# YHY138/Boosting-Fine-grained-Feature-Fusion-in-3D-Point-Cloud-Registration

Measured on AMD Instinct MI355X. Metric: point-cloud pairs/sec (forward) on ModelNet 2048-pt pairs, higher is better.
Workload: dtype f32 (emulated on the fp16 MFMA pipe: f16x3 split products); 1 GPU; ModelNet40 2048-pt pairs, 8 pairs per GPU (BASELINE configs[1] at N=1, configs[3] at N=8); pairs_per_gpu=8, global_batch=8, points_per_cloud=717, parallelism=pair-sharded dp1, precision=fp32

## Files before the change

### boosting-fine-grained-feature-fusion-in-3d-point-cloud-registration_amd/csrc/res2net.hip

```cpp
#include "mfma.h"

namespace fgr {
namespace {

constexpr int kCpU = 8;
__device__ __forceinline__ void copy_rows(float* __restrict__ dst, int64_t ldd,
                                          const float* __restrict__ src, int64_t lds, int64_t r0,
                                          int rows, int64_t n, int cols, int tid, int nth) {
    const bool v4 = ((cols | (int)(ldd & 3) | (int)(lds & 3)) & 3) == 0 &&
                    ((reinterpret_cast<uintptr_t>(dst) | reinterpret_cast<uintptr_t>(src)) & 15) == 0;
    if (v4) {
        const int c4 = cols / 4;
        const int nr = (int)min<int64_t>(rows, n - r0);
        if (nr <= 0 || c4 == 0) return;
        const int tot = nr * c4;
        for (int e0 = tid; e0 < tot; e0 += kCpU * nth) {
            float4 v[kCpU];
#pragma unroll
            for (int u = 0; u < kCpU; ++u) {
                const int e = min(e0 + u * nth, tot - 1);
                const int row = e / c4, cc = (e - row * c4) * 4;
                v[u] = *reinterpret_cast<const float4*>(src + (r0 + row) * lds + cc);
            }
#pragma unroll
// ... 226 lines not shown
                ah[f] = __builtin_bit_cast(f16x8, img[0 * NU + base + 16 * f + c]);
                am[f] = __builtin_bit_cast(f16x8, img[1 * NU + base + 16 * f + c]);
            }
#pragma unroll
            for (int f = 0; f < RF; ++f) acc[f] = __builtin_amdgcn_mfma_f32_16x16x32_f16(wl, ah[f], acc[f], 0, 0, 0);
#pragma unroll
            for (int f = 0; f < RF; ++f) acc[f] = __builtin_amdgcn_mfma_f32_16x16x32_f16(wh, am[f], acc[f], 0, 0, 0);
#pragma unroll
            for (int f = 0; f < RF; ++f) acc[f] = __builtin_amdgcn_mfma_f32_16x16x32_f16(wh, ah[f], acc[f], 0, 0, 0);
        }
#pragma unroll
        for (int rg = 0; rg < RF; ++rg) {
            const int row = rg * 16 + c;
            const float mx = __int_as_float(rm[row]);
            const float rs = __builtin_ldexpf(1.f, mx > 0.f ? -row_scale_exp(mx) : 0);
            const f32x4 av = acc[rg];
            float4 y;
            y.x = fmaxf(av[0] * rs * wsv.x + bc.x, 0.f);
            y.y = fmaxf(av[1] * rs * wsv.y + bc.y, 0.f);
            y.z = fmaxf(av[2] * rs * wsv.z + bc.z, 0.f);
            y.w = fmaxf(av[3] * rs * wsv.w + bc.w, 0.f);
            if (r0 + row < n && col_ok)
                *reinterpret_cast<float4*>(cat + (r0 + row) * ld + (int64_t)i * w + col0) = y;
            *reinterpret_cast<float4*>(sp + row * SPW + col0) = y;
        }
        if (tid < R) rmax[(i + 1) & 1][tid] = 0;
        __syncthreads();
    }
    copy_rows(cat + (int64_t)nums * w, ld, h + (int64_t)nums * w, hw, r0, R, n,
              (scale - nums) * w, tid, nth);
    if (x) copy_rows(cat + hw, ld, x, cin, r0, R, n, cin, tid, nth);
}

}
}

using namespace fgr;

extern "C" int fgr_res2net_chain_h3(const float* h, int64_t n, int32_t w, int32_t scale,
                                    const void* w_img, const float* w_scale, const float* bias,
                                    const float* x, int32_t cin, float* cat, int64_t ld_cat,
                                    void* stream) {
    FGR_REQUIRE(n >= 0 && scale >= 2 && w > 0 && w <= 224 && w % 4 == 0 && cin >= 0,
                "fgr_res2net_chain_h3: unsupported width %d / scale %d (w %% 4 == 0, <= 224)", w,
                scale);
    FGR_REQUIRE(ld_cat >= (int64_t)scale * w + (x ? cin : 0) && ld_cat % 4 == 0,
                "fgr_res2net_chain_h3: ld_cat too small or not a multiple of 4");
    FGR_REQUIRE(n == 0 || (h && w_img && w_scale && bias && cat), "fgr_res2net_chain_h3: null pointer");
    FGR_REQUIRE(((reinterpret_cast<uintptr_t>(h) | reinterpret_cast<uintptr_t>(cat) |
                  reinterpret_cast<uintptr_t>(w_scale) | reinterpret_cast<uintptr_t>(bias)) & 15) == 0 &&
                    (scale * w) % 4 == 0,
                "fgr_res2net_chain_h3: h / cat / w_scale / bias must be 16-B aligned");
    if (n == 0) return FGR_OK;
    hipStream_t st = as_stream(stream);
    TimedCall timed_(st);
    const int kt = (w + 15) / 16;
    const char* rr = getenv("FGR_R2N_ROWS");
    const bool r48 = kt == 14 && !(rr && rr[0] == '3') &&
                     ceil_div(ceil_div(n, 48), 256) * 48 < ceil_div(ceil_div(n, 32), 256) * 32;
#define FGR_H3_CASE(KT)                                                                         \
    case KT:                                                                                    \
        hipLaunchKernelGGL(res2net_chain_h3_kernel<KT>, dim3((unsigned)ceil_div(n, kRows)),     \
                           dim3(64 * KT), 0, st, h, n, w, scale, scale - 1, (const u32x4*)w_img, \
                           w_scale, bias, x, cin, cat, ld_cat);                                 \
        break;
    if (r48) {
        hipLaunchKernelGGL((res2net_chain_h3_kernel<14, 48>), dim3((unsigned)ceil_div(n, 48)),
                           dim3(64 * 14), 0, st, h, n, w, scale, scale - 1, (const u32x4*)w_img,
                           w_scale, bias, x, cin, cat, ld_cat);
        FGR_CHECK_LAUNCH("res2net_chain_h3_kernel");
// ... 20 lines not shown
                "fgr_res2net_chain6: unsupported width %d / scale %d (needs 112 or 224)", w, scale);
    FGR_REQUIRE(ld_cat >= (int64_t)scale * w + (x ? cin : 0), "fgr_res2net_chain6: ld_cat too small");
    FGR_REQUIRE(n == 0 || (h && w_img && bias && cat), "fgr_res2net_chain6: null pointer");
    FGR_REQUIRE(((reinterpret_cast<uintptr_t>(h) & 15) == 0) && (scale * w) % 4 == 0,
                "fgr_res2net_chain6: h must be 16-B aligned");
    if (n == 0) return FGR_OK;
    hipStream_t st = as_stream(stream);
    TimedCall timed_(st);
    const char* rr = getenv("FGR_R2N_ROWS");
    int rows = 32;
    if (w == 224 && !(rr && rr[0] == '3')) {
        int64_t best = ceil_div(ceil_div(n, 32), 256) * 32;
        for (int r : {48, 16}) {
            const int64_t cost = ceil_div(ceil_div(n, r), 256) * r;
            if (cost < best) { best = cost; rows = r; }
        }
    }
    const int64_t b32 = ceil_div(n, 32);
    if (w == 112)
        hipLaunchKernelGGL(res2net_chain6_kernel<7>, dim3((unsigned)b32), dim3(64 * 7), 0, st, h, n,
                           scale, scale - 1, (const u32x4*)w_img, bias, x, cin, cat, ld_cat);
    else if (rows == 48)
        hipLaunchKernelGGL((res2net_chain6_kernel<14, 48>), dim3((unsigned)ceil_div(n, 48)), dim3(64 * 14),
                           0, st, h, n, scale, scale - 1, (const u32x4*)w_img, bias, x, cin, cat, ld_cat);
    else if (rows == 16)
        hipLaunchKernelGGL((res2net_chain6_kernel<14, 16>), dim3((unsigned)ceil_div(n, 16)), dim3(64 * 14),
                           0, st, h, n, scale, scale - 1, (const u32x4*)w_img, bias, x, cin, cat, ld_cat);
    else
        hipLaunchKernelGGL(res2net_chain6_kernel<14>, dim3((unsigned)b32), dim3(64 * 14), 0, st, h, n,
                           scale, scale - 1, (const u32x4*)w_img, bias, x, cin, cat, ld_cat);
    FGR_CHECK_LAUNCH("res2net_chain6_kernel");
    return FGR_OK;
}
```

### boosting-fine-grained-feature-fusion-in-3d-point-cloud-registration_amd/fgreg/_lib.py

```python
import ctypes
import os
import subprocess

HERE = os.path.dirname(os.path.abspath(__file__))
LIB_PATH = os.environ.get('FGREG_LIB_PATH') or os.path.join(HERE, 'libfgreg.so')
CSRC = os.path.join(os.path.dirname(HERE), 'csrc')

_vp = ctypes.c_void_p
_i32 = ctypes.c_int32
_i64 = ctypes.c_int64
_f32 = ctypes.c_float
_sz = ctypes.c_size_t

ABI_VERSION = 2

SIGNATURES = {
    'fgr_grid_subsample_workspace': [_i64, _i32, _i64, ctypes.POINTER(_sz)],
    'fgr_grid_subsample_count': [_vp, _vp, _i32, _i64, _f32, _i64, _vp, _sz, _vp, _vp],
    'fgr_grid_subsample_fill': [_i64, _i32, _i64, _i64, _vp, _sz, _vp, _vp, _vp, _vp],
    'fgr_radius_grid_workspace': [_i64, _i32, ctypes.POINTER(_sz)],
    'fgr_radius_grid_build': [_vp, _vp, _i32, _i64, _f32, _vp, _sz, _vp],
    'fgr_radius_search_grid': [_vp, _vp, _i32, _i64, _i32, _vp, _vp, _i64, _vp, _sz, _f32, _i32,
                               _i32, _vp, _vp, _vp, _vp],
    'fgr_radius_count': [_vp, _vp, _vp, _vp, _i32, _i64, _i32, _f32, _vp, _vp, _vp],
# ... 6 lines not shown
    'fgr_kpconv_deform_points': [_vp, _vp, _vp, _vp, _i64, _i32, _f32, _vp, _vp, _vp],
    'fgr_kpconv_gather_deform_workspace': [_i64, _i32, ctypes.POINTER(_sz)],
    'fgr_kpconv_gather_deform': [_vp, _vp, _i64, _i64, _vp, _i32, _vp, _i32, _vp, _vp, _i32, _f32,
                                 _i32, _i32, _vp, _vp, _vp, _sz, _vp],
    'fgr_kpconv_scatter_deform_workspace': [_i64, _i32, _i32, ctypes.POINTER(_sz)],
    'fgr_kpconv_scatter_deform': [_vp, _vp, _i64, _i64, _vp, _i32, _vp, _i32, _vp, _vp, _i32, _f32,
                                  _i32, _i32, _vp, _vp, _vp, _vp, _sz, _vp],
    'fgr_kpconv_deform_grad': [_vp, _vp, _i64, _i64, _vp, _i32, _vp, _i32, _vp, _vp, _vp, _i32,
                               _f32, _i32, _i32, _vp, _vp, _vp],
    'fgr_max_pool': [_vp, _i64, _i32, _vp, _i64, _i32, _vp, _vp],
    'fgr_instnorm_workspace': [_i64, _i32, _i32, ctypes.POINTER(_sz)],
    'fgr_instnorm': [_vp, _i64, _i32, _vp, _i32, _i64, _vp, _f32, _i32, _vp, _i32, _vp, _vp, _sz,
                     _vp],
    'fgr_layernorm': [_vp, _i64, _i32, _vp, _vp, _f32, _vp, _vp, _vp, _vp],
    'fgr_sine_pos_embed': [_vp, _i64, _i32, _f32, _f32, _vp, _vp],
    'fgr_add': [_vp, _vp, _i64, _vp, _vp],
    'fgr_layernorm_dual': [_vp, _i64, _i32, _vp, _vp, _vp, _vp, _vp, _vp, _vp, _vp, _f32, _vp],
    'fgr_attention': [_vp, _i64, _vp, _i64, _vp, _i64, _vp, _i64, _vp, _vp, _vp, _i32, _i32, _i32,
                      _i32, _f32, _vp],
    'fgr_attention_f16x3_workspace': [_i64, _i32, _i32, ctypes.POINTER(_sz)],
    'fgr_attention_f16x3': [_vp, _i64, _vp, _i64, _vp, _i64, _vp, _i64, _vp, _vp, _vp, _i32, _i32,
                            _i64, _i32, _i32, _i32, _i32, _f32, _vp, _i64, _vp],
    'fgr_attention_f16x3_drop': [_vp, _i64, _vp, _i64, _vp, _i64, _vp, _i64, _vp, _vp, _vp, _i32,
                                 _i32, _i64, _i32, _i32, _i32, _i32, _f32, _vp, _i64,
                                 ctypes.c_uint32, _f32, _vp],
    'fgr_attention_f16x3_train': [_vp, _i64, _vp, _i64, _vp, _i64, _vp, _i64, _vp, _vp, _vp, _i32,
                                  _i32, _i64, _i32, _i32, _i32, _i32, _f32, _vp, _i64,
                                  ctypes.c_uint32, _f32, _vp, _vp],
    'fgr_attention_bf16_workspace': [_i64, _i32, _i32, ctypes.POINTER(_sz)],
    'fgr_attention_bf16': [_vp, _i64, _vp, _i64, _vp, _i64, _vp, _i64, _vp, _vp, _vp, _i32, _i32,
                           _i64, _i32, _i32, _i32, _i32, _f32, _vp, _i64, _vp],
    'fgr_res2net_chain6': [_vp, _i64, _i32, _i32, _vp, _vp, _vp, _i32, _vp, _i64, _vp],
    'fgr_res2net_chain_h3': [_vp, _i64, _i32, _i32, _vp, _vp, _vp, _vp, _i32, _vp, _i64, _vp],
    'fgr_split_weights_h3_bytes': [_i32, _i32, ctypes.POINTER(_sz)],
    'fgr_split_weights_h3_batch': [_vp, _i32, _i64, _vp],
    'fgr_split_weights_h3': [_vp, _i32, _i32, _i64, _i64, _vp, _vp],
    'fgr_gemm_f16x3': [_vp, _i64, _vp, _vp, _i64, _vp, _vp, _i64, _i32, _i32, _i32, _i32, _vp],
    'fgr_gemm_f16x3_ln_supported': [_i32, _i32, _i32],
    'fgr_gemm_f16x3_ln': [_vp, _i64, _vp, _vp, _f32, _vp, _i64, _vp, _vp, _i64, _vp, _i32, _i32,
                          _i32, _i32, _vp],
    'fgr_gemm_f16x3_ln_out2': [_vp, _i64, _vp, _vp, _f32, _vp, _i64, _vp, _vp, _i64, _vp, _i32,
                               _i32, _i32, _i32, _vp, _vp, _vp, _i64, _vp],
    'fgr_split_weights_ffn2_bytes': [_i32, _i32, ctypes.POINTER(_sz)],
    'fgr_split_weights_ffn2': [_vp, _i32, _i32, _i64, _i64, _vp, _vp],
    'fgr_ffn_f16x3_supported': [_i32, _i32, _i32],
    'fgr_ffn_f16x3': [_vp, _i64, _vp, _vp, _f32, _vp, _vp, _vp, _vp, _vp, _vp, _i64, _i32, _i32,
                      _i32, _vp],
    'fgr_ffn_f16x3_act_supported': [_i32, _i32, _i32, _i32],
    'fgr_ffn_f16x3_act': [_vp, _i64, _vp, _vp, _f32, _vp, _vp, _vp, _vp, _vp, _vp, _i64, _i32,
                          _i32, _i32, _i32, _vp],
    'fgr_gelu_fwd': [_vp, _vp, _i64, _vp],
    'fgr_gelu_bwd': [_vp, _vp, _vp, _i64, _vp],
    'fgr_pos_mlp_f16x3_supported': [_i64, _i32],
    'fgr_pos_mlp_f16x3': [_vp, _i64, _vp, _vp, _vp, _vp, _vp, _vp, _vp, _vp, _vp, _vp, _i32, _vp,
                          _i64, _vp],
    'fgr_split_weights_bf16_bytes': [_i32, _i32, ctypes.POINTER(_sz)],
    'fgr_split_weights_bf16': [_vp, _i32, _i32, _i64, _i64, _vp, _vp],
    'fgr_gemm_bf16': [_vp, _i64, _vp, _vp, _i64, _vp, _vp, _i64, _i32, _i32, _i32, _i32, _vp],
    'fgr_gemm_workspace': [_i32, _i32, _i32, _i32, ctypes.POINTER(_sz)],
    'fgr_gemm_f16x3_ws': [_vp, _i64, _vp, _vp, _i64, _vp, _vp, _i64, _i32, _i32, _i32, _i32, _vp,
                          _sz, _vp],
    'fgr_gemm_bf16_ws': [_vp, _i64, _vp, _vp, _i64, _vp, _vp, _i64, _i32, _i32, _i32, _i32, _vp,
                         _sz, _vp],
    'fgr_kv_image_bytes': [_i64, _i32, _i32, ctypes.POINTER(_sz)],
    'fgr_gemm_f16x3_ln_qkv_supported': [_i32, _i32, _i32],
    'fgr_gemm_f16x3_ln_qkv': [_vp, _i64, _vp, _vp, _f32, _vp, _i64, _vp, _vp, _i64, _vp, _i32, _i32,
# ... 136 lines not shown
```

### boosting-fine-grained-feature-fusion-in-3d-point-cloud-registration_amd/fgreg/backbone.py

```python
import math
import os
from typing import List

import numpy as np

import torch
import torch.nn as nn
import torch.nn.functional as F

from . import linear as lin
from . import ops
from .linear import linear


class PreprocessorHIP(nn.Module):

    def __init__(self, cfg, neighbor_mode='ball_query'):
        super().__init__()
        self.cfg = cfg
        self.mode = {'ball_query': ops.NB_INDEX, 'nanoflann': ops.NB_DIST}[neighbor_mode]

    def _lengths_to_device(self, lens, device):
        if device.type != 'cuda':
            return torch.tensor(lens, dtype=torch.int64, device=device)
        buf = getattr(self, '_pin', None)
        if buf is None or buf.numel() < len(lens):
            buf = torch.empty(max(64, len(lens)), dtype=torch.int64, pin_memory=True)
            self._pin, self._pin_ev = buf, None
        if self._pin_ev is not None:
            self._pin_ev.synchronize()
        buf[:len(lens)].copy_(torch.tensor(lens, dtype=torch.int64))
        out = buf[:len(lens)].to(device, non_blocking=True)
        self._pin_ev = torch.cuda.Event()
        self._pin_ev.record()
        return out

    def forward(self, pts: List[torch.Tensor]):
        cfg = self.cfg
        limits = cfg.neighborhood_limits
        device = pts[0].device
        r_normal = cfg.first_subsampling_dl * cfg.conv_radius
        arch = cfg.architecture
        lens = [int(p.shape[0]) for p in pts]
        points = torch.cat([p.float() for p in pts], 0).contiguous()
        len_dev = self._lengths_to_device(lens, device)
# ... 234 lines not shown
        self.conv3 = nn.Linear(width * scale, planes, bias=False)
        self.bn3 = nn.BatchNorm1d(planes)
        self.downsample = downsample
        self.stype, self.scale, self.width = stype, scale, width
        self._folded = None

    @staticmethod
    def _fold(lin, bn):
        s = bn.weight / torch.sqrt(bn.running_var + bn.eps)
        return (lin.weight * s[:, None]).contiguous(), (bn.bias - bn.running_mean * s).contiguous()

    def _folded_params(self):
        key = tuple((p._version, p.data_ptr()) for p in self.parameters()) + tuple(
            (b._version, b.data_ptr()) for b in self.buffers())
        if self._folded is None or self._folded[0] != key:
            with torch.no_grad():
                w1, b1 = self._fold(self.conv1, self.bn1)
                ws = [self._fold(c, b) for c, b in zip(self.convs, self.bns)]
                w3, b3 = self._fold(self.conv3, self.bn3)
                if self.downsample is not None:
                    wd, bd = self._fold(self.downsample[0], self.downsample[1])
                    w3d = torch.cat([w3, wd], 1).contiguous()
                    b3d = (b3 + bd).contiguous()
                else:
                    w3d, b3d = w3, b3
                chain = None
                if w1.is_cuda and self.nums > 0 and self.downsample is not None:
                    wst = torch.stack([wi for wi, _ in ws])
                    bst = torch.stack([bi for _, bi in ws]).contiguous()
                    if self.width == 224 and os.environ.get('FGREG_R2N224', 'x6') != 'h3':
                        chain = (bst, ops.res2net_fragments3(wst), None)
                    elif ops.res2net_chain_supported(self.width, True):
                        chain = (bst,) + ops.res2net_fragments_h3(wst)
            self._folded = (key, w1, b1, ws, w3d, b3d, chain)
            ops.note_state(w1, b1, w3d, b3d, *[t for wb in ws for t in wb],
                           *(chain if chain is not None else ()))
        return self._folded[1:]

    def forward(self, x, shortcut=None):
        if self.training:
            from .training import bottle2neck_train
            y = bottle2neck_train(self, x)
            return y if shortcut is None else F.leaky_relu(y + shortcut, 0.1)
        w1, b1, ws, w3d, b3d, chain = self._folded_params()
        out = linear(x, w1, b1, act=ops.ACT_RELU)
        w = self.width
        down = self.downsample is not None
        cat_in = torch.empty((x.shape[0], w * self.scale + (x.shape[1] if down else 0)),
                             dtype=x.dtype, device=x.device)
        if chain is not None:
            ops.res2net_chain(out, w, self.scale, chain[1], chain[0], x, cat_in, w_scale=chain[2])
        else:
            sp = None
            for i in range(self.nums):
                chunk = out[:, i * w:(i + 1) * w]
                sp = chunk if i == 0 else sp + chunk
                sp = linear(sp, ws[i][0], ws[i][1], act=ops.ACT_RELU,
                            out=cat_in[:, i * w:(i + 1) * w])
            if self.scale != 1:
                cat_in[:, self.nums * w:self.scale * w] = out[:, self.nums * w:self.scale * w]
            if down:
                cat_in[:, self.scale * w:] = x
        if down:
            if shortcut is not None:
                return linear(cat_in, w3d, b3d, act=ops.ACT_RELU_RES_LEAKY, residual=shortcut)
            return linear(cat_in, w3d, b3d, act=ops.ACT_RELU)
        y = linear(cat_in, w3d, b3d, act=ops.ACT_RELU, residual=x)
        return y if shortcut is None else F.leaky_relu(y + shortcut, 0.1)


class my_res2Net(nn.Module):
    def __init__(self, block, in_dim, out_dim, baseWidth=26, scale=4):
        super().__init__()
        downsample = None
        if in_dim != out_dim * block.expansion:
            downsample = nn.Sequential(nn.Linear(in_dim, out_dim, bias=False),
                                       nn.BatchNorm1d(out_dim))
        self.layer1 = nn.Sequential(block(in_dim, out_dim, 1, downsample=downsample,
                                          stype='normal', baseWidth=baseWidth, scale=scale))

    def forward(self, x, shortcut=None):
        return self.layer1(x) if shortcut is None else self.layer1[0](x, shortcut)

# ... 111 lines not shown
```

### boosting-fine-grained-feature-fusion-in-3d-point-cloud-registration_amd/fgreg/ops.py

```python
import ctypes
import math
from typing import Optional, Sequence, Tuple

import torch

from . import _lib
from ._lib import (ACT_GELU, ACT_LEAKY, ACT_NONE, ACT_RELU, ACT_RELU_RES_LEAKY,
                   NB_DIST, NB_INDEX)


def _ptr(t):
    return None if t is None else t.data_ptr()


class KernelTimer:

    def __init__(self, names):
        self.names = set(names)
        self.events = {n: [] for n in names}
        self.work = {n: [] for n in names}
        self.labels = {n: [] for n in names}
        self.count = False
        self.pool = []
        self.lead_cycles = 0
# ... 491 lines not shown
    wp[:, :w, :w] = weights * sc[..., None]
    hi = wp.to(torch.float16)
    lo = (wp - hi.float()).to(torch.float16)
    t = torch.stack([hi, lo], 0).reshape(2, nums, wp_rows // 16, 16, ks, 4, 8)
    img = t.permute(1, 2, 4, 0, 5, 3, 6).contiguous()
    return img, (1.0 / sc).contiguous()


def res2net_chain_supported(w, h3=False):
    if h3:
        return w % 4 == 0 and (w + 15) // 16 in (2, 4, 7, 14)
    return w in (112, 224)


def res2net_chain(h, w, scale, w_frag, bias, x, cat, w_scale=None):
    _dev(h, w_frag, w_scale, bias, x, cat)
    h = _c(h, torch.float32)
    n = h.shape[0]
    assert h.shape[1] == scale * w and cat.shape[0] == n and cat.stride(1) == 1
    cin = 0 if x is None else x.shape[1]
    if x is not None:
        x = _c(x, torch.float32)
    L = _lib.load()
    t0 = _begin('res2net', 'h3' if w_scale is not None else 'x6')
    work = 2 * n * w * w * (scale - 1) * (3 if w_scale is not None else 6)
    if w_scale is not None:
        _lib.check(L.fgr_res2net_chain_h3(
            _ptr(h), n, w, scale, _ptr(w_frag), _ptr(w_scale), _ptr(bias), _ptr(x), cin,
            _ptr(cat), cat.stride(0), _stream()), 'fgr_res2net_chain_h3')
    else:
        _lib.check(L.fgr_res2net_chain6(_ptr(h), n, w, scale, _ptr(w_frag), _ptr(bias), _ptr(x),
                                        cin, _ptr(cat), cat.stride(0), _stream()),
                   'fgr_res2net_chain6')
    _end('res2net', t0, work)
    return cat


ATTN_MODE = 'f16x3'


def attention(q, k, v, q_off, kv_off, kv_seg, max_q_len, n_head, out=None,
              max_kv_len=None, dropout=None, lse=None) -> torch.Tensor:
    _dev(q, k, v, q_off, kv_off, kv_seg)
    for t in (q, k, v):
        assert t.dtype == torch.float32 and t.dim() == 2 and t.stride(1) == 1
    d = q.shape[1]
    assert k.shape[1] == d and v.shape[1] == d and d % n_head == 0 and k.shape[0] == v.shape[0]
    dh = d // n_head
    if out is None:
        out = torch.empty((q.shape[0], d), dtype=torch.float32, device=q.device)
    n_seg = q_off.numel() - 1
    n_kv_seg = kv_off.numel() - 1
    assert kv_seg.dtype == torch.int32 and kv_seg.numel() == n_seg
    max_kv_len = max_q_len if max_kv_len is None else max_kv_len
    L = _lib.load()
    split = (dh in (32, 64)
             and all(t.stride(0) % 4 == 0 and t.data_ptr() % 16 == 0 for t in (q, k, v, out)))
    t0 = _begin('attention')
    if lse is not None:
        assert split and ATTN_MODE == 'f16x3' and lse.is_contiguous() and lse.shape == (q.shape[0], n_head)
        seed, p = (int(dropout[0]), float(dropout[1])) if dropout is not None else (0, 0.0)
        nb = _lib.ws_size('fgr_attention_f16x3_workspace', k.shape[0], n_kv_seg, n_head)
        ws = _workspace(q.device, nb)
        _lib.check(L.fgr_attention_f16x3_train(
            _ptr(q), q.stride(0), _ptr(k), k.stride(0), _ptr(v), v.stride(0), _ptr(out),
            out.stride(0), _ptr(q_off), _ptr(kv_off), _ptr(kv_seg), n_seg, n_kv_seg, k.shape[0],
# ... 346 lines not shown
```

### include/fgreg.h

```cpp
#ifndef FGREG_H
#define FGREG_H

#include <stddef.h>
#include <stdint.h>

#ifdef __cplusplus
extern "C" {
#endif

#define FGR_ABI_VERSION 2

enum {
    FGR_OK = 0,
    FGR_E_ARG = -1,
    FGR_E_LAUNCH = -2,
    FGR_E_WORKSPACE = -3
};

enum {
    FGR_NB_INDEX = 0,
    FGR_NB_DIST = 1
};

enum { FGR_ACT_NONE = 0, FGR_ACT_LEAKY = 1, FGR_ACT_RELU = 2, FGR_ACT_RELU_RES_LEAKY = 3,
// ... 69 lines not shown
                           float* d_mod, void* stream);

int fgr_max_pool(const float* x, int64_t ns, int32_t c, const int64_t* idx, int64_t nq,
                 int32_t width, float* out, void* stream);

int fgr_instnorm_workspace(int64_t max_seg_len, int32_t c, int32_t n_seg, size_t* bytes);
int fgr_instnorm(const float* x, int64_t n, int32_t c, const int64_t* seg_off, int32_t n_seg,
                 int64_t max_seg_len, const float* row_div, float eps, int32_t act,
                 const float* residual, int32_t post_act, float* out, void* ws, size_t ws_bytes,
                 void* stream);

int fgr_layernorm(float* x, int64_t n, int32_t d, const float* gamma, const float* beta,
                  float eps, const float* add, const float* pre_bias, float* out, void* stream);
int fgr_layernorm_dual(const float* x, int64_t n, int32_t d, const float* gamma,
                       const float* beta, const float* add, float* out, const float* gamma2,
                       const float* beta2, const float* add2, float* out2, float eps,
                       void* stream);

int fgr_add(const float* a, const float* b, int64_t n, float* out, void* stream);

int fgr_gelu_fwd(const float* z, float* y, int64_t n, void* stream);
int fgr_gelu_bwd(const float* z, const float* dy, float* dz, int64_t n, void* stream);

int fgr_sine_pos_embed(const float* xyz, int64_t n, int32_t d_model, float temperature,
                       float scale, float* out, void* stream);

int fgr_res2net_chain6(const float* h, int64_t n, int32_t w, int32_t scale, const void* w_img,
                       const float* bias, const float* x, int32_t cin, float* cat,
                       int64_t ld_cat, void* stream);

int fgr_res2net_chain_h3(const float* h, int64_t n, int32_t w, int32_t scale, const void* w_img,
                         const float* w_scale, const float* bias, const float* x, int32_t cin,
                         float* cat, int64_t ld_cat, void* stream);

int fgr_split_weights_h3_bytes(int32_t n, int32_t k, size_t* bytes);
int fgr_split_weights_h3(const float* w, int32_t n, int32_t k, int64_t stride_n,
                         int64_t stride_k, void* img, void* stream);
typedef struct {
    const float* w;
    void* img;
    int64_t stride_n;
    int64_t stride_k;
    int64_t panel0;
    int32_t n;
    int32_t k;
} fgr_split_desc;
int fgr_split_weights_h3_batch(const void* descs, int32_t count, int64_t total_panels,
                               void* stream);
int fgr_gemm_f16x3(const float* a, int64_t lda, const void* w_img, float* c, int64_t ldc,
                   const float* bias, const float* r, int64_t ldr, int32_t m, int32_t n,
                   int32_t k, int32_t act, void* stream);

int fgr_gemm_workspace(int32_t m, int32_t n, int32_t k, int32_t mode, size_t* bytes);
int fgr_gemm_f16x3_ws(const float* a, int64_t lda, const void* w_img, float* c, int64_t ldc,
                      const float* bias, const float* r, int64_t ldr, int32_t m, int32_t n,
                      int32_t k, int32_t act, void* ws, size_t ws_bytes, void* stream);
int fgr_gemm_bf16_ws(const float* a, int64_t lda, const void* w_img, float* c, int64_t ldc,
                     const float* bias, const float* r, int64_t ldr, int32_t m, int32_t n,
                     int32_t k, int32_t act, void* ws, size_t ws_bytes, void* stream);

int fgr_gemm_f16x3_ln_supported(int32_t m, int32_t n, int32_t k);
int fgr_gemm_f16x3_ln(const float* x, int64_t ldx, const float* gamma, const float* beta,
                      float eps, const float* add, int64_t ld_add, const void* w_img, float* c,
                      int64_t ldc, const float* bias, int32_t m, int32_t n, int32_t k,
                      int32_t act, void* stream);
int fgr_gemm_f16x3_ln_out2(const float* x, int64_t ldx, const float* gamma, const float* beta,
// ... 254 lines not shown
```

Before: 3221 pairs/s.

## Fuse Res2Net conv1 into the hierarchical split-conv chain kernel

```diff
diff --git a/boosting-fine-grained-feature-fusion-in-3d-point-cloud-registration_amd/csrc/res2net.hip b/boosting-fine-grained-feature-fusion-in-3d-point-cloud-registration_amd/csrc/res2net.hip
--- a/boosting-fine-grained-feature-fusion-in-3d-point-cloud-registration_amd/csrc/res2net.hip
+++ b/boosting-fine-grained-feature-fusion-in-3d-point-cloud-registration_amd/csrc/res2net.hip
@@ -282,10 +282,510 @@
     if (x) copy_rows(cat + hw, ld, x, cin, r0, R, n, cin, tid, nth);
 }
 
+template <int KT, int KSX, int R = kRows>
+__global__ void __launch_bounds__(64 * KT, KT == 7 ? 4 : 1)
+res2net_block_h3_kernel(const float* __restrict__ x, int64_t n, int w, int scale,
+                        const u32x4* __restrict__ w1f, const float* __restrict__ w1sc,
+                        const float* __restrict__ b1, const u32x4* __restrict__ wf,
+                        const float* __restrict__ wsc, const float* __restrict__ bias,
+                        float* __restrict__ cat, int64_t ld) {
+    constexpr int W = 16 * KT, KS = (W + 31) / 32, NU = R * KS * 4, NTH = 64 * KT;
+    constexpr int CIN = 32 * KSX, NUX = R * KSX * 4;
+    constexpr int IT = (NU + NTH - 1) / NTH, ITX = (NUX + NTH - 1) / NTH;
+    constexpr int RF = R / 16, SPW = W + 4;
+    __shared__ u32x4 img[2 * NU];
+    __shared__ u32x4 ximg[2 * NUX];
+    __shared__ float sp[R * SPW];
+    __shared__ int rmax[2][R];
+    __shared__ int xmax[R];
+    const int tid = threadIdx.x;
+    const int wv = tid / 64, lane = tid % 64, g = lane >> 4, c = lane & 15;
+    const int64_t r0 = (int64_t)blockIdx.x * R;
+    const int64_t hw = (int64_t)scale * w;
+    const int nums = scale - 1;
+    const int col0 = wv * 16 + 4 * g;
+    const bool col_ok = col0 < w;
+    if (tid < R) { rmax[0][tid] = 0; rmax[1][tid] = 0; xmax[tid] = 0; }
+
+    u32x4 w1q[KSX][2];
+    float4 w1sv, b1v;
+    auto load_w1 = [&](int j) {
+        const u32x4* wb = w1f + (((int64_t)j * KT + wv) * KSX) * 128 + lane;
+#pragma unroll
+        for (int q = 0; q < KSX; ++q)
+#pragma unroll
+            for (int t = 0; t < 2; ++t) w1q[q][t] = wb[(q * 2 + t) * 64];
+        w1sv = b1v = make_float4(0.f, 0.f, 0.f, 0.f);
+        if (col_ok) {
+            w1sv = ld4(w1sc + (int64_t)j * w + col0);
+            b1v = ld4(b1 + (int64_t)j * w + col0);
+        }
+    };
+    load_w1(0);
+    __syncthreads();
+
+    {
+        float xa[ITX][8];
+#pragma unroll
+        for (int it = 0; it < ITX; ++it) {
+            const int u = tid + NTH * it;
+            const int row = u % R, kg = u / R;
+            const int64_t gr = r0 + row;
+#pragma unroll
+            for (int e = 0; e < 8; e += 4) {
+                float4 v = make_float4(0.f, 0.f, 0.f, 0.f);
+                if (u < NUX && gr < n) v = ld4(x + gr * CIN + 8 * kg + e);
+                xa[it][e] = v.x; xa[it][e + 1] = v.y; xa[it][e + 2] = v.z; xa[it][e + 3] = v.w;
+            }
+        }
+#pragma unroll
+        for (int it = 0; it < ITX; ++it) {
+            const int u = tid + NTH * it;
+            const int row = u % R, kg = u / R;
+            const int64_t gr = r0 + row;
+            if (u < NUX && gr < n) {
+                float* d = cat + gr * ld + hw + 8 * kg;
+                *reinterpret_cast<float4*>(d) = make_float4(xa[it][0], xa[it][1], xa[it][2], xa[it][3]);
+                *reinterpret_cast<float4*>(d + 4) = make_float4(xa[it][4], xa[it][5], xa[it][6], xa[it][7]);
+            }
+            float cm = 0.f;
+#pragma unroll
+            for (int e = 0; e < 8; ++e) cm = fmaxf(cm, fabsf(xa[it][e]));
+            if (u < NUX && cm > 0.f) atomicMax(&xmax[row], __float_as_int(cm));
+        }
+        __syncthreads();
+#pragma unroll
+        for (int it = 0; it < ITX; ++it) {
+            const int u = tid + NTH * it;
+            if (u >= NUX) break;
+            const int row = u % R, kg = u / R;
+            const float s = __builtin_ldexpf(1.f, row_scale_exp(__int_as_float(xmax[row])));
+            f16x8 th, tm;
+#pragma unroll
+            for (int e = 0; e < 8; ++e) {
+                const float xs = xa[it][e] * s;
+                const _Float16 hh = (_Float16)xs;
+                th[e] = hh;
+                tm[e] = (_Float16)(xs - (float)hh);
+            }
+            ximg[0 * NUX + kg * R + row] = __builtin_bit_cast(u32x4, th);
+            ximg[1 * NUX + kg * R + row] = __builtin_bit_cast(u32x4, tm);
+        }
+    }
+    __syncthreads();
+    float rsx[RF];
+#pragma unroll
+    for (int rg = 0; rg < RF; ++rg) {
+        const float mx = __int_as_float(xmax[rg * 16 + c]);
+        rsx[rg] = __builtin_ldexpf(1.f, mx > 0.f ? -row_scale_exp(mx) : 0);
+    }
+    f32x4 acc1[RF];
+    auto conv1_step = [&](int ks) {
+        const f16x8 wh = __builtin_bit_cast(f16x8, w1q[ks][0]);
+        const f16x8 wl = __builtin_bit_cast(f16x8, w1q[ks][1]);
+        const int base = (ks * 4 + g) * R;
+        f16x8 xh[RF], xl[RF];
+#pragma unroll
+        for (int f = 0; f < RF; ++f) {
+            xh[f] = __builtin_bit_cast(f16x8, ximg[0 * NUX + base + 16 * f + c]);
+            xl[f] = __builtin_bit_cast(f16x8, ximg[1 * NUX + base + 16 * f + c]);
+        }
+#pragma unroll
+        for (int f = 0; f < RF; ++f) acc1[f] = __builtin_amdgcn_mfma_f32_16x16x32_f16(wl, xh[f], acc1[f], 0, 0, 0);
+#pragma unroll
+        for (int f = 0; f < RF; ++f) acc1[f] = __builtin_amdgcn_mfma_f32_16x16x32_f16(wh, xl[f], acc1[f], 0, 0, 0);
+#pragma unroll
+        for (int f = 0; f < RF; ++f) acc1[f] = __builtin_amdgcn_mfma_f32_16x16x32_f16(wh, xh[f], acc1[f], 0, 0, 0);
+    };
+    auto conv1_out = [&](const f32x4 av, const int rg) {
+        float4 hv;
+        hv.x = fmaxf(av[0] * (rsx[rg] * w1sv.x) + b1v.x, 0.f);
+        hv.y = fmaxf(av[1] * (rsx[rg] * w1sv.y) + b1v.y, 0.f);
+        hv.z = fmaxf(av[2] * (rsx[rg] * w1sv.z) + b1v.z, 0.f);
+        hv.w = fmaxf(av[3] * (rsx[rg] * w1sv.w) + b1v.w, 0.f);
+        return hv;
+    };
+    auto put_a = [&](const float4& a, int row, int* rm) {
+        *reinterpret_cast<float4*>(sp + row * SPW + col0) = a;
+        const float cm = fmaxf(fmaxf(a.x, a.y), fmaxf(a.z, a.w));
+        if (cm > 0.f) atomicMax(&rm[row], __float_as_int(cm));
+    };
+
+    {
+#pragma unroll
+        for (int f = 0; f < RF; ++f) acc1[f] = f32x4{0.f, 0.f, 0.f, 0.f};
+#pragma unroll
+        for (int ks = 0; ks < KSX; ++ks) conv1_step(ks);
+#pragma unroll
+        for (int rg = 0; rg < RF; ++rg) put_a(conv1_out(acc1[rg], rg), rg * 16 + c, rmax[0]);
+    }
+    __syncthreads();
+
+    for (int i = 0; i < nums; ++i) {
+        int* rm = rmax[i & 1];
+        int* rmn = rmax[(i + 1) & 1];
+        const u32x4* wb = wf + (((int64_t)i * KT + wv) * KS) * 128 + lane;
+        u32x4 bq[KS][2];
+#pragma unroll
+        for (int q = 0; q < KS; ++q)
+#pragma unroll
+            for (int t = 0; t < 2; ++t) bq[q][t] = wb[(q * 2 + t) * 64];
+        float4 wsv = make_float4(0.f, 0.f, 0.f, 0.f), bc = wsv;
+        if (col_ok) {
+            wsv = ld4(wsc + i * w + col0);
+            bc = ld4(bias + i * w + col0);
+        }
+        load_w1(i + 1);
+        if (tid < R) rmn[tid] = 0;
+#pragma unroll
+        for (int it = 0; it < IT; ++it) {
+            const int u = tid + NTH * it;
+            if (u >= NU) break;
+            const int row = u % R, kg = u / R, k0 = 8 * kg;
+            float a[8] = {0.f, 0.f, 0.f, 0.f, 0.f, 0.f, 0.f, 0.f};
+            if (k0 < W) {
+                const float4 s0 = *reinterpret_cast<const float4*>(sp + row * SPW + k0);
+                const float4 s1 = *reinterpret_cast<const float4*>(sp + row * SPW + k0 + 4);
+                a[0] = s0.x; a[1] = s0.y; a[2] = s0.z; a[3] = s0.w;
+                a[4] = s1.x; a[5] = s1.y; a[6] = s1.z; a[7] = s1.w;
+            }
+            const float s = __builtin_ldexpf(1.f, row_scale_exp(__int_as_float(rm[row])));
+            f16x8 th, tm;
+#pragma unroll
+            for (int e = 0; e < 8; ++e) {
+                const float xs = a[e] * s;
+                const _Float16 hh = (_Float16)xs;
+                th[e] = hh;
+                tm[e] = (_Float16)(xs - (float)hh);
+            }
+            img[0 * NU + kg * R + row] = __builtin_bit_cast(u32x4, th);
+            img[1 * NU + kg * R + row] = __builtin_bit_cast(u32x4, tm);
+        }
+#pragma unroll
+        for (int f = 0; f < RF; ++f) acc1[f] = f32x4{0.f, 0.f, 0.f, 0.f};
+#pragma unroll
+        for (int ks = 0; ks < KSX; ++ks) conv1_step(ks);
+        __syncthreads();
+        f32x4 acc[RF];
+#pragma unroll
+        for (int f = 0; f < RF; ++f) acc[f] = f32x4{0.f, 0.f, 0.f, 0.f};
+#pragma unroll
+        for (int ks = 0; ks < KS; ++ks) {
+            const f16x8 wh = __builtin_bit_cast(f16x8, bq[ks][0]);
+            const f16x8 wl = __builtin_bit_cast(f16x8, bq[ks][1]);
+            const int base = (ks * 4 + g) * R;
+            f16x8 ah[RF], am[RF];
+#pragma unroll
+            for (int f = 0; f < RF; ++f) {
+                ah[f] = __builtin_bit_cast(f16x8, img[0 * NU + base + 16 * f + c]);
+                am[f] = __builtin_bit_cast(f16x8, img[1 * NU + base + 16 * f + c]);
+            }
+#pragma unroll
+            for (int f = 0; f < RF; ++f) acc[f] = __builtin_amdgcn_mfma_f32_16x16x32_f16(wl, ah[f], acc[f], 0, 0, 0);
+#pragma unroll
+            for (int f = 0; f < RF; ++f) acc[f] = __builtin_amdgcn_mfma_f32_16x16x32_f16(wh, am[f], acc[f], 0, 0, 0);
+#pragma unroll
+            for (int f = 0; f < RF; ++f) acc[f] = __builtin_amdgcn_mfma_f32_16x16x32_f16(wh, ah[f], acc[f], 0, 0, 0);
+        }
+#pragma unroll
+        for (int rg = 0; rg < RF; ++rg) {
+            const int row = rg * 16 + c;
+            const float mx = __int_as_float(rm[row]);
+            const float rs = __builtin_ldexpf(1.f, mx > 0.f ? -row_scale_exp(mx) : 0);
+            const f32x4 av = acc[rg];
+            float4 y;
+            y.x = fmaxf(av[0] * rs * wsv.x + bc.x, 0.f);
+            y.y = fmaxf(av[1] * rs * wsv.y + bc.y, 0.f);
+            y.z = fmaxf(av[2] * rs * wsv.z + bc.z, 0.f);
+            y.w = fmaxf(av[3] * rs * wsv.w + bc.w, 0.f);
+            const float4 hv = conv1_out(acc1[rg], rg);
+            const bool st = r0 + row < n && col_ok;
+            float* crow = cat + (r0 + row) * ld + col0;
+            if (st) *reinterpret_cast<float4*>(crow + (int64_t)i * w) = y;
+            if (i + 1 < nums)
+                put_a(make_float4(y.x + hv.x, y.y + hv.y, y.z + hv.z, y.w + hv.w), row, rmn);
+            else if (st)
+                *reinterpret_cast<float4*>(crow + (int64_t)(i + 1) * w) = hv;
+        }
+        __syncthreads();
+    }
+}
+
+template <int KT, int KSX, int R = kRows>
+__global__ void __launch_bounds__(64 * KT)
+res2net_block6_kernel(const float* __restrict__ x, int64_t n, int scale,
+                      const u32x4* __restrict__ w1f, const float* __restrict__ w1sc,
+                      const float* __restrict__ b1, const u32x4* __restrict__ wf,
+                      const float* __restrict__ bias, float* __restrict__ cat, int64_t ld) {
+    constexpr int W = 16 * KT, KS = (W + 31) / 32, NU = R * KS * 4, NTH = 64 * KT;
+    constexpr int CIN = 32 * KSX, NUX = R * KSX * 4;
+    constexpr int ITX = (NUX + NTH - 1) / NTH;
+    constexpr int RF = R / 16, SPW = W + 4;
+    __shared__ u32x4 img[3 * NU];
+    __shared__ u32x4 ximg[2 * NUX];
+    __shared__ float sp[R * SPW];
+    __shared__ int xmax[R];
+    __shared__ float xrs[R];
+    const int tid = threadIdx.x;
+    const int wv = tid / 64, lane = tid % 64, g = lane >> 4, c = lane & 15;
+    const int64_t r0 = (int64_t)blockIdx.x * R;
+    const int64_t hw = (int64_t)scale * W;
+    const int nums = scale - 1;
+    const int col = wv * 16 + c;
+    if (tid < R) xmax[tid] = 0;
+    __syncthreads();
+
+    {
+        float xa[ITX][8];
+#pragma unroll
+        for (int it = 0; it < ITX; ++it) {
+            const int u = tid + NTH * it;
+            const int row = u % R, kg = u / R;
+            const int64_t gr = r0 + row;
+#pragma unroll
+            for (int e = 0; e < 8; e += 4) {
+                float4 v = make_float4(0.f, 0.f, 0.f, 0.f);
+                if (u < NUX && gr < n) v = ld4(x + gr * CIN + 8 * kg + e);
+                xa[it][e] = v.x; xa[it][e + 1] = v.y; xa[it][e + 2] = v.z; xa[it][e + 3] = v.w;
+            }
+        }
+#pragma unroll
+        for (int it = 0; it < ITX; ++it) {
+            const int u = tid + NTH * it;
+            const int row = u % R, kg = u / R;
+            const int64_t gr = r0 + row;
+            if (u < NUX && gr < n) {
+                float* d = cat + gr * ld + hw + 8 * kg;
+                *reinterpret_cast<float4*>(d) = make_float4(xa[it][0], xa[it][1], xa[it][2], xa[it][3]);
+                *reinterpret_cast<float4*>(d + 4) = make_float4(xa[it][4], xa[it][5], xa[it][6], xa[it][7]);
+            }
+            float cm = 0.f;
+#pragma unroll
+            for (int e = 0; e < 8; ++e) cm = fmaxf(cm, fabsf(xa[it][e]));
+            if (u < NUX && cm > 0.f) atomicMax(&xmax[row], __float_as_int(cm));
+        }
+        __syncthreads();
+        if (tid < R) xrs[tid] = __builtin_ldexpf(1.f, -row_scale_exp(__int_as_float(xmax[tid])));
+#pragma unroll
+        for (int it = 0; it < ITX; ++it) {
+            const int u = tid + NTH * it;
+            if (u >= NUX) break;
+            const int row = u % R, kg = u / R;
+            const float s = __builtin_ldexpf(1.f, row_scale_exp(__int_as_float(xmax[row])));
+            f16x8 th, tm;
+#pragma unroll
+            for (int e = 0; e < 8; ++e) {
+                const float xs = xa[it][e] * s;
+                const _Float16 hh = (_Float16)xs;
+                th[e] = hh;
+                tm[e] = (_Float16)(xs - (float)hh);
+            }
+            ximg[0 * NUX + kg * R + row] = __builtin_bit_cast(u32x4, th);
+            ximg[1 * NUX + kg * R + row] = __builtin_bit_cast(u32x4, tm);
+        }
+    }
+    __syncthreads();
+
+    u32x4 w1q[2][2];
+    auto w1_base = [&](int j) { return w1f + (((int64_t)j * KT + wv) * KSX) * 128 + lane; };
+    auto w1_head = [&](const u32x4* wb) {
+#pragma unroll
+        for (int q = 0; q < 2; ++q)
+            if (q < KSX) {
+#pragma unroll
+                for (int t = 0; t < 2; ++t) w1q[q][t] = wb[(q * 2 + t) * 64];
+            }
+    };
+    f32x4 acc1[RF];
+    auto conv1 = [&](const u32x4* wb) {
+#pragma unroll
+        for (int f = 0; f < RF; ++f) acc1[f] = f32x4{0.f, 0.f, 0.f, 0.f};
+#pragma unroll
+        for (int ks = 0; ks < KSX; ++ks) {
+            const f16x8 wh = __builtin_bit_cast(f16x8, w1q[ks % 2][0]);
+            const f16x8 wl = __builtin_bit_cast(f16x8, w1q[ks % 2][1]);
+            const int base = (ks * 4 + g) * R;
+            f16x8 xh[RF], xl[RF];
+#pragma unroll
+            for (int f = 0; f < RF; ++f) {
+                xh[f] = __builtin_bit_cast(f16x8, ximg[0 * NUX + base + 16 * f + c]);
+                xl[f] = __builtin_bit_cast(f16x8, ximg[1 * NUX + base + 16 * f + c]);
+            }
+#pragma unroll
+            for (int f = 0; f < RF; ++f) acc1[f] = __builtin_amdgcn_mfma_f32_16x16x32_f16(xh[f], wl, acc1[f], 0, 0, 0);
+#pragma unroll
+            for (int f = 0; f < RF; ++f) acc1[f] = __builtin_amdgcn_mfma_f32_16x16x32_f16(xl[f], wh, acc1[f], 0, 0, 0);
+#pragma unroll
+            for (int f = 0; f < RF; ++f) acc1[f] = __builtin_amdgcn_mfma_f32_16x16x32_f16(xh[f], wh, acc1[f], 0, 0, 0);
+            if (ks + 2 < KSX) {
+#pragma unroll
+                for (int t = 0; t < 2; ++t) w1q[ks % 2][t] = wb[((ks + 2) * 2 + t) * 64];
+            }
+        }
+    };
+    auto conv1_out = [&](const float a, const int row, const float ws, const float bb) {
+        return fmaxf(a * (xrs[row] * ws) + bb, 0.f);
+    };
+
+    {
+        const u32x4* wb = w1_base(0);
+        w1_head(wb);
+        const float ws = w1sc[col], bb = b1[col];
+        conv1(wb);
+#pragma unroll
+        for (int rg = 0; rg < RF; ++rg)
+#pragma unroll
+            for (int r = 0; r < 4; ++r) {
+                const int row = rg * 16 + 4 * g + r;
+                sp[row * SPW + col] = conv1_out(acc1[rg][r], row, ws, bb);
+            }
+    }
+    __syncthreads();
+
+    for (int i = 0; i < nums; ++i) {
+        const u32x4* wb = wf + (((int64_t)i * KT + wv) * KS) * 192 + lane;
+        u32x4 bq[3][3];
+#pragma unroll
+        for (int q = 0; q < 2; ++q)
+            if (q < KS) {
+#pragma unroll
+                for (int t = 0; t < 3; ++t) bq[q][t] = wb[(q * 3 + t) * 64];
+            }
+        const float bc = bias[i * W + col];
+        const u32x4* wb1 = w1_base(i + 1);
+        w1_head(wb1);
+        const float ws = w1sc[(i + 1) * W + col], bb = b1[(i + 1) * W + col];
+        auto build = [&](const int u) {
+            const int row = u % R, kg = u / R;
+            const int k0 = 8 * kg;
+            float a[8] = {0.f, 0.f, 0.f, 0.f, 0.f, 0.f, 0.f, 0.f};
+            if (W % 32 == 0 || k0 < W) {
+                const float4 s0 = *reinterpret_cast<const float4*>(sp + row * SPW + k0);
+                const float4 s1 = *reinterpret_cast<const float4*>(sp + row * SPW + k0 + 4);
+                a[0] = s0.x; a[1] = s0.y; a[2] = s0.z; a[3] = s0.w;
+                a[4] = s1.x; a[5] = s1.y; a[6] = s1.z; a[7] = s1.w;
+            }
+            bf16x8 th, tm, tl;
+#pragma unroll
+            for (int e = 0; e < 8; ++e) {
+                __bf16 hh, mm, ll;
+                split3(a[e], hh, mm, ll);
+                th[e] = hh; tm[e] = mm; tl[e] = ll;
+            }
+            img[0 * NU + kg * R + row] = __builtin_bit_cast(u32x4, th);
+            img[1 * NU + kg * R + row] = __builtin_bit_cast(u32x4, tm);
+            img[2 * NU + kg * R + row] = __builtin_bit_cast(u32x4, tl);
+        };
+        constexpr int IT = (NU + NTH - 1) / NTH;
+#pragma unroll
+        for (int it = 0; it < IT; ++it) {
+            const int u = tid + NTH * it;
+            if ((it + 1) * NTH <= NU || u < NU) build(u);
+        }
+        conv1(wb1);
+        __syncthreads();
+        f32x4 acc[RF];
+#pragma unroll
+        for (int f = 0; f < RF; ++f) acc[f] = f32x4{0.f, 0.f, 0.f, 0.f};
+#pragma unroll
+        for (int ks = 0; ks < KS; ++ks) {
+            if (ks + 2 < KS) {
+#pragma unroll
+                for (int t = 0; t < 3; ++t) bq[(ks + 2) % 3][t] = wb[((ks + 2) * 3 + t) * 64];
+            }
+            const bf16x8 bh = __builtin_bit_cast(bf16x8, bq[ks % 3][0]);
+            const bf16x8 bm = __builtin_bit_cast(bf16x8, bq[ks % 3][1]);
+            const bf16x8 bl = __builtin_bit_cast(bf16x8, bq[ks % 3][2]);
+            const int base = (ks * 4 + g) * R;
+            bf16x8 ah[RF], am[RF], al[RF];
+#pragma unroll
+            for (int f = 0; f < RF; ++f) {
+                ah[f] = __builtin_bit_cast(bf16x8, img[0 * NU + base + 16 * f + c]);
+                am[f] = __builtin_bit_cast(bf16x8, img[1 * NU + base + 16 * f + c]);
+                al[f] = __builtin_bit_cast(bf16x8, img[2 * NU + base + 16 * f + c]);
+            }
+#pragma unroll
+            for (int f = 0; f < RF; ++f) acc[f] = __builtin_amdgcn_mfma_f32_16x16x32_bf16(am[f], bm, acc[f], 0, 0, 0);
+#pragma unroll
+            for (int f = 0; f < RF; ++f) acc[f] = __builtin_amdgcn_mfma_f32_16x16x32_bf16(al[f], bh, acc[f], 0, 0, 0);
+#pragma unroll
+            for (int f = 0; f < RF; ++f) acc[f] = __builtin_amdgcn_mfma_f32_16x16x32_bf16(ah[f], bl, acc[f], 0, 0, 0);
+#pragma unroll
+            for (int f = 0; f < RF; ++f) acc[f] = __builtin_amdgcn_mfma_f32_16x16x32_bf16(am[f], bh, acc[f], 0, 0, 0);
+#pragma unroll
+            for (int f = 0; f < RF; ++f) acc[f] = __builtin_amdgcn_mfma_f32_16x16x32_bf16(ah[f], bm, acc[f], 0, 0, 0);
+#pragma unroll
+            for (int f = 0; f < RF; ++f) acc[f] = __builtin_amdgcn_mfma_f32_16x16x32_bf16(ah[f], bh, acc[f], 0, 0, 0);
+        }
+#pragma unroll
+        for (int rg = 0; rg < RF; ++rg) {
+#pragma unroll
+            for (int r = 0; r < 4; ++r) {
+                const int row = rg * 16 + 4 * g + r;
+                const float y = fmaxf(acc[rg][r] + bc, 0.f);
+                const float hv = conv1_out(acc1[rg][r], row, ws, bb);
+                float* crow = cat + (r0 + row) * ld + col;
+                if (r0 + row < n) crow[(int64_t)i * W] = y;
+                if (i + 1 < nums) sp[row * SPW + col] = y + hv;
+                else if (r0 + row < n) crow[(int64_t)(i + 1) * W] = hv;
+            }
+        }
+        __syncthreads();
+    }
+}
+
 }
 }
 
 using namespace fgr;
+
+static int block_h3_kt(int w, int cin) {
+    const int kt = (w + 15) / 16;
+    if (w <= 0 || w % 4 != 0) return 0;
+    if ((kt == 2 && cin == 32) || (kt == 4 && cin == 64) || (kt == 7 && cin == 128)) return kt;
+    return 0;
+}
+
+extern "C" int fgr_res2net_block_h3(const float* x, int64_t n, int32_t w, int32_t cin,
+                                    int32_t scale, const void* w1_img, const float* w1_scale,
+                                    const float* b1, const void* w_img, const float* w_scale,
+                                    const float* bias, float* cat, int64_t ld_cat, void* stream) {
+    FGR_REQUIRE(n >= 0 && scale >= 2, "fgr_res2net_block_h3: bad n %lld / scale %d", (long long)n,
+                scale);
+    const int kt = block_h3_kt(w, cin);
+    FGR_REQUIRE(kt != 0,
+                "fgr_res2net_block_h3: no instance for width %d with cin %d ((28, 32), (56, 64), "
+                "(112, 128) up to tile padding)", w, cin);
+    FGR_REQUIRE(ld_cat >= (int64_t)scale * w + cin && ld_cat % 4 == 0,
+                "fgr_res2net_block_h3: ld_cat %lld too small (needs %lld) or not a multiple of 4",
+                (long long)ld_cat, (long long)scale * w + cin);
+    FGR_REQUIRE(n == 0 || (x && w1_img && w1_scale && b1 && w_img && w_scale && bias && cat),
+                "fgr_res2net_block_h3: null pointer");
+    const uintptr_t al = reinterpret_cast<uintptr_t>(x) | reinterpret_cast<uintptr_t>(cat) |
+                         reinterpret_cast<uintptr_t>(w1_scale) | reinterpret_cast<uintptr_t>(b1) |
+                         reinterpret_cast<uintptr_t>(w_scale) | reinterpret_cast<uintptr_t>(bias) |
+                         reinterpret_cast<uintptr_t>(w1_img) | reinterpret_cast<uintptr_t>(w_img);
+    FGR_REQUIRE((al & 15) == 0,
+                "fgr_res2net_block_h3: x %p / cat %p / images / scales / biases must be 16-B aligned",
+                (const void*)x, (const void*)cat);
+    if (n == 0) return FGR_OK;
+    hipStream_t st = as_stream(stream);
+    TimedCall timed_(st);
+#define FGR_BH3_CASE(KT, KSX)                                                                    \
+    case KT:                                                                                     \
+        hipLaunchKernelGGL((res2net_block_h3_kernel<KT, KSX>), dim3((unsigned)ceil_div(n, kRows)), \
+                           dim3(64 * KT), 0, st, x, n, w, scale, (const u32x4*)w1_img, w1_scale, \
+                           b1, (const u32x4*)w_img, w_scale, bias, cat, ld_cat);                 \
+        break;
+    switch (kt) {
+        FGR_BH3_CASE(2, 1)
+        FGR_BH3_CASE(4, 2)
+        FGR_BH3_CASE(7, 4)
+    }
+#undef FGR_BH3_CASE
+    FGR_CHECK_LAUNCH("res2net_block_h3_kernel");
+    return FGR_OK;
+}
 
 extern "C" int fgr_res2net_chain_h3(const float* h, int64_t n, int32_t w, int32_t scale,
                                     const void* w_img, const float* w_scale, const float* bias,
@@ -372,3 +872,44 @@
     FGR_CHECK_LAUNCH("res2net_chain6_kernel");
     return FGR_OK;
 }
+
+extern "C" int fgr_res2net_block6(const float* x, int64_t n, int32_t w, int32_t cin, int32_t scale,
+                                  const void* w1_img, const float* w1_scale, const float* b1,
+                                  const void* w_img, const float* bias, float* cat,
+                                  int64_t ld_cat, void* stream) {
+    FGR_REQUIRE(n >= 0 && scale >= 2, "fgr_res2net_block6: bad n %lld / scale %d", (long long)n,
+                scale);
+    FGR_REQUIRE(w == 224 && cin == 256,
+                "fgr_res2net_block6: no instance for width %d with cin %d (needs 224, 256)", w, cin);
+    FGR_REQUIRE(ld_cat >= (int64_t)scale * w + cin && ld_cat % 4 == 0,
+                "fgr_res2net_block6: ld_cat %lld too small (needs %lld) or not a multiple of 4",
+                (long long)ld_cat, (long long)scale * w + cin);
+    FGR_REQUIRE(n == 0 || (x && w1_img && w1_scale && b1 && w_img && bias && cat),
+                "fgr_res2net_block6: null pointer");
+    const uintptr_t al = reinterpret_cast<uintptr_t>(x) | reinterpret_cast<uintptr_t>(cat) |
+                         reinterpret_cast<uintptr_t>(w1_img) | reinterpret_cast<uintptr_t>(w_img);
+    FGR_REQUIRE((al & 15) == 0, "fgr_res2net_block6: x %p / cat %p / images must be 16-B aligned",
+                (const void*)x, (const void*)cat);
+    if (n == 0) return FGR_OK;
+    hipStream_t st = as_stream(stream);
+    TimedCall timed_(st);
+    const char* rr = getenv("FGR_R2N_ROWS");
+    int rows = 32;
+    if (!(rr && rr[0] == '3')) {
+        int64_t best = ceil_div(ceil_div(n, 32), 256) * 32;
+        for (int r : {48, 16}) {
+            const int64_t cost = ceil_div(ceil_div(n, r), 256) * r;
+            if (cost < best) { best = cost; rows = r; }
+        }
+    }
+#define FGR_B6_LAUNCH(R)                                                                        \
+    hipLaunchKernelGGL((res2net_block6_kernel<14, 8, R>), dim3((unsigned)ceil_div(n, R)),       \
+                       dim3(64 * 14), 0, st, x, n, scale, (const u32x4*)w1_img, w1_scale, b1,   \
+                       (const u32x4*)w_img, bias, cat, ld_cat)
+    if (rows == 48) FGR_B6_LAUNCH(48);
+    else if (rows == 16) FGR_B6_LAUNCH(16);
+    else FGR_B6_LAUNCH(32);
+#undef FGR_B6_LAUNCH
+    FGR_CHECK_LAUNCH("res2net_block6_kernel");
+    return FGR_OK;
+}
diff --git a/boosting-fine-grained-feature-fusion-in-3d-point-cloud-registration_amd/fgreg/_lib.py b/boosting-fine-grained-feature-fusion-in-3d-point-cloud-registration_amd/fgreg/_lib.py
--- a/boosting-fine-grained-feature-fusion-in-3d-point-cloud-registration_amd/fgreg/_lib.py
+++ b/boosting-fine-grained-feature-fusion-in-3d-point-cloud-registration_amd/fgreg/_lib.py
@@ -62,6 +62,9 @@
                            _i64, _i32, _i32, _i32, _i32, _f32, _vp, _i64, _vp],
     'fgr_res2net_chain6': [_vp, _i64, _i32, _i32, _vp, _vp, _vp, _i32, _vp, _i64, _vp],
     'fgr_res2net_chain_h3': [_vp, _i64, _i32, _i32, _vp, _vp, _vp, _vp, _i32, _vp, _i64, _vp],
+    'fgr_res2net_block_h3': [_vp, _i64, _i32, _i32, _i32, _vp, _vp, _vp, _vp, _vp, _vp, _vp, _i64,
+                             _vp],
+    'fgr_res2net_block6': [_vp, _i64, _i32, _i32, _i32, _vp, _vp, _vp, _vp, _vp, _vp, _i64, _vp],
     'fgr_split_weights_h3_bytes': [_i32, _i32, ctypes.POINTER(_sz)],
     'fgr_split_weights_h3_batch': [_vp, _i32, _i64, _vp],
     'fgr_split_weights_h3': [_vp, _i32, _i32, _i64, _i64, _vp, _vp],
diff --git a/boosting-fine-grained-feature-fusion-in-3d-point-cloud-registration_amd/fgreg/backbone.py b/boosting-fine-grained-feature-fusion-in-3d-point-cloud-registration_amd/fgreg/backbone.py
--- a/boosting-fine-grained-feature-fusion-in-3d-point-cloud-registration_amd/fgreg/backbone.py
+++ b/boosting-fine-grained-feature-fusion-in-3d-point-cloud-registration_amd/fgreg/backbone.py
@@ -11,6 +11,8 @@
 from . import linear as lin
 from . import ops
 from .linear import linear
+
+R2N_FUSED = True
 
 
 class PreprocessorHIP(nn.Module):
@@ -311,6 +313,9 @@
                         chain = (bst, ops.res2net_fragments3(wst), None)
                     elif ops.res2net_chain_supported(self.width, True):
                         chain = (bst,) + ops.res2net_fragments_h3(wst)
+                    if chain is not None and ops.res2net_block_supported(
+                            self.width, w1.shape[1], chain[2] is not None):
+                        chain = chain + ops.res2net_conv1_fragments(w1, self.scale)
             self._folded = (key, w1, b1, ws, w3d, b3d, chain)
             ops.note_state(w1, b1, w3d, b3d, *[t for wb in ws for t in wb],
                            *(chain if chain is not None else ()))
@@ -322,12 +327,17 @@
             y = bottle2neck_train(self, x)
             return y if shortcut is None else F.leaky_relu(y + shortcut, 0.1)
         w1, b1, ws, w3d, b3d, chain = self._folded_params()
-        out = linear(x, w1, b1, act=ops.ACT_RELU)
         w = self.width
         down = self.downsample is not None
         cat_in = torch.empty((x.shape[0], w * self.scale + (x.shape[1] if down else 0)),
                              dtype=x.dtype, device=x.device)
-        if chain is not None:
+        fused = R2N_FUSED and chain is not None and len(chain) == 5 and lin.MODE == 'f16x3'
+        if not fused:
+            out = linear(x, w1, b1, act=ops.ACT_RELU)
+        if fused:
+            ops.res2net_block(x, w, self.scale, chain[3], chain[4], b1, chain[1], chain[0],
+                              cat_in, w_scale=chain[2])
+        elif chain is not None:
             ops.res2net_chain(out, w, self.scale, chain[1], chain[0], x, cat_in, w_scale=chain[2])
         else:
             sp = None
diff --git a/boosting-fine-grained-feature-fusion-in-3d-point-cloud-registration_amd/fgreg/ops.py b/boosting-fine-grained-feature-fusion-in-3d-point-cloud-registration_amd/fgreg/ops.py
--- a/boosting-fine-grained-feature-fusion-in-3d-point-cloud-registration_amd/fgreg/ops.py
+++ b/boosting-fine-grained-feature-fusion-in-3d-point-cloud-registration_amd/fgreg/ops.py
@@ -547,6 +547,55 @@
         _lib.check(L.fgr_res2net_chain6(_ptr(h), n, w, scale, _ptr(w_frag), _ptr(bias), _ptr(x),
                                         cin, _ptr(cat), cat.stride(0), _stream()),
                    'fgr_res2net_chain6')
+    _end('res2net', t0, work)
+    return cat
+
+
+def res2net_conv1_fragments(w1: torch.Tensor, scale: int = 1):
+    rows, cin = w1.shape
+    w = rows // scale
+    assert rows == scale * w and cin % 32 == 0
+    kt = (w + 15) // 16
+    mx = w1.abs().amax(dim=1)
+    e = torch.where(mx > 0, 15 - torch.frexp(mx).exponent, torch.zeros_like(mx, dtype=torch.int32))
+    e = e.clamp(max=127)
+    sc = torch.ldexp(torch.ones_like(mx), e.float())
+    wp = torch.zeros((scale, kt * 16, cin), dtype=torch.float32, device=w1.device)
+    wp[:, :w] = (w1 * sc[:, None]).reshape(scale, w, cin)
+    hi = wp.to(torch.float16)
+    lo = (wp - hi.float()).to(torch.float16)
+    t = torch.stack([hi, lo], 0).reshape(2, scale * kt, 16, cin // 32, 4, 8)
+    img = t.permute(1, 3, 0, 4, 2, 5).contiguous()
+    return img, (1.0 / sc).contiguous()
+
+
+def res2net_block_supported(w, cin, h3=True):
+    if not h3:
+        return (w, cin) == (224, 256)
+    return w > 0 and w % 4 == 0 and ((w + 15) // 16, cin) in ((2, 32), (4, 64), (7, 128))
+
+
+def res2net_block(x, w, scale, w1_img, w1_scale, b1, w_frag, bias, cat, w_scale=None):
+    _dev(x, w1_img, w1_scale, b1, w_frag, w_scale, bias, cat)
+    x = _c(x, torch.float32)
+    n, cin = x.shape
+    h3 = w_scale is not None
+    if not res2net_block_supported(w, cin, h3):
+        raise _lib.FgrError(f'res2net_block: no fused instance for w {w}, cin {cin}, '
+                            f'{"f16x3" if h3 else "bf16x6"}')
+    assert cat.shape[0] == n and cat.stride(1) == 1
+    L = _lib.load()
+    t0 = _begin('res2net', 'h3' if h3 else 'x6')
+    work = 2 * n * w * w * (scale - 1) * (3 if h3 else 6) + 3 * 2 * n * cin * scale * w
+    if h3:
+        _lib.check(L.fgr_res2net_block_h3(
+            _ptr(x), n, w, cin, scale, _ptr(w1_img), _ptr(w1_scale), _ptr(b1), _ptr(w_frag),
+            _ptr(w_scale), _ptr(bias), _ptr(cat), cat.stride(0), _stream()),
+            'fgr_res2net_block_h3')
+    else:
+        _lib.check(L.fgr_res2net_block6(
+            _ptr(x), n, w, cin, scale, _ptr(w1_img), _ptr(w1_scale), _ptr(b1), _ptr(w_frag),
+            _ptr(bias), _ptr(cat), cat.stride(0), _stream()), 'fgr_res2net_block6')
     _end('res2net', t0, work)
     return cat
 
diff --git a/include/fgreg.h b/include/fgreg.h
--- a/include/fgreg.h
+++ b/include/fgreg.h
@@ -125,6 +125,16 @@
 int fgr_res2net_chain_h3(const float* h, int64_t n, int32_t w, int32_t scale, const void* w_img,
                          const float* w_scale, const float* bias, const float* x, int32_t cin,
                          float* cat, int64_t ld_cat, void* stream);
+
+int fgr_res2net_block_h3(const float* x, int64_t n, int32_t w, int32_t cin, int32_t scale,
+                         const void* w1_img, const float* w1_scale, const float* b1,
+                         const void* w_img, const float* w_scale, const float* bias, float* cat,
+                         int64_t ld_cat, void* stream);
+
+int fgr_res2net_block6(const float* x, int64_t n, int32_t w, int32_t cin, int32_t scale,
+                       const void* w1_img, const float* w1_scale, const float* b1,
+                       const void* w_img, const float* bias, float* cat, int64_t ld_cat,
+                       void* stream);
 
 int fgr_split_weights_h3_bytes(int32_t n, int32_t k, size_t* bytes);
 int fgr_split_weights_h3(const float* w, int32_t n, int32_t k, int64_t stride_n,
```

Measured after the change: 3305 pairs/s, median of 6. +2.6%, better.
